# Isomorpfishm/SINGA

Measured on AMD Instinct MI355X. Metric: protein-ligand graphs/sec GAN step (G+D fwd+bwd); scatter-TP kernel HBM GB/s, higher is better.
Workload: dtype f32

## Files before the change

### __graft_entry__.py

```python
import os
import subprocess
import sys

ROOT = os.path.dirname(os.path.abspath(__file__))
if ROOT not in sys.path:
    sys.path.insert(0, ROOT)

SRC = os.path.join(ROOT, "singa_amd", "csrc", "singa_hip.hip")
LIB = os.path.join(ROOT, "singa_amd", "lib", "libsinga_hip.so")


def build() -> None:
    os.makedirs(os.path.dirname(LIB), exist_ok=True)
    deps = [SRC, os.path.join(ROOT, "singa_amd", "csrc", "so3_index.h"), os.path.join(ROOT, "include", "singa_hip.h"),
            os.path.join(ROOT, "include", "singa_hip_lab.h"), os.path.join(ROOT, "include", "singa_hip_gen.h"),
            os.path.join(ROOT, "include", "singa_hip_force.h"), os.path.join(ROOT, "include", "singa_hip_swor.h"),
            os.path.join(ROOT, "include", "singa_hip_stream.h"), os.path.join(ROOT, "include", "singa_hip_valence.h"),
            os.path.join(ROOT, "include", "singa_hip_beam.h"), os.path.join(ROOT, "include", "singa_hip_units.h"),
            os.path.join(ROOT, "include", "singa_hip_prefix.h"), os.path.join(ROOT, "include", "singa_hip_data.h"),
            os.path.join(ROOT, "include", "singa_hip_attn_tiles.h"), os.path.join(ROOT, "include", "singa_hip_bf16.h"),
            os.path.join(ROOT, "include", "singa_hip_dec_tiles.h")]
    if not os.path.exists(LIB) or any(os.path.getmtime(d) > os.path.getmtime(LIB) for d in deps):
        hipcc = os.environ.get("HIPCC", "/opt/rocm/bin/hipcc")
        cmd = [hipcc, "--offload-arch=gfx950", "-O3", "-std=c++17", "-shared", "-fPIC", "-o", LIB, SRC]
        subprocess.check_call(cmd)
    import torch
    import singa_amd
    from singa_amd import _capi
    _capi.bind(LIB)


def smoke() -> None:
    import numpy as np
    import torch

    build()
    from oracle import singa_oracle as O
    from singa_amd import graph as G
    from singa_amd.config import load_config
    from singa_amd.model.GAN import SINGA
    from tests.helpers import golden, state_from_spec

    assert torch.cuda.is_available(), "smoke() needs a GPU"
    L = 2
    dev = "cuda:0"
    sd = state_from_spec(f"singa_L{L}")
    z = golden(f"singa_L{L}_B3.npz")
    names = ["3wi2_4tpp", "4agq_5a7b", "5cp5_4nue"]
    batch = G.collate([G.load_npz(os.path.join(ROOT, "tests", "golden", f"graph_{n}.npz"), with_lap=False) for n in names])
    batch.nodes[G.PA]["lap_pe"], batch.nodes[G.LA]["lap_pe"] = torch.tensor(z["lap_p"]), torch.tensor(z["lap_l"])
    batch.extras["edge_rot_mat"] = {k: torch.tensor(z[f"rot_{k}"]) for k in ("pp", "ll", "lp")}
    batch.extras["knn"] = {G.PA: torch.tensor(z["knn_p"]), G.LA: torch.tensor(z["knn_l"])}
    batch = batch.to(dev)
    model = SINGA(load_config(lmax=L), device=dev)
    model.load_state_dict(sd, strict=False)
    model.eval()
    logits = model(batch)
    loss = torch.nn.functional.cross_entropy(logits, batch["ligand_data"]["smiIndices_tgt"].reshape(-1))
    loss.backward()
    torch.cuda.synchronize()
    og = O.collate([O.load_graph_npz(os.path.join(ROOT, "tests", "golden", f"graph_{n}.npz")) for n in names])
    rots = {k: torch.as_tensor(z[f"rot_{k}"]) for k in ("pp", "ll", "lp")}
    with torch.no_grad():
        ref = O.singa_forward(sd, og, rots, L, torch.as_tensor(z["knn_p"]), torch.as_tensor(z["knn_l"]),
                              torch.as_tensor(z["lap_p"]), torch.as_tensor(z["lap_l"]))
    err = float((logits.detach().cpu().double() - ref.double()).norm() / ref.double().norm())
    gn = float(torch.sqrt(sum((p.grad.double() ** 2).sum() for p in model.parameters() if p.grad is not None)))
    print(f"smoke: loss {float(loss):.6f} (reference {float(z['loss']):.6f}), logits rel err vs oracle {err:.2e}, "
          f"grad norm {gn:.4f} (reference {float(z['grad_total']):.4f})")
    assert err < 1e-4, err
    assert abs(gn - float(z["grad_total"])) < 1e-4 * float(z["grad_total"])


if __name__ == "__main__":
    build()
    if len(sys.argv) > 1 and sys.argv[1] == "smoke":
        smoke()
```

### singa_amd/_capi.py

```python
import ctypes as C

P = C.c_void_p
I32 = C.c_int
I64 = C.c_int64
F32 = C.c_float


class Seg(C.Structure):
    _fields_ = [("ptr", P), ("ld", I64), ("rows", C.c_int32)]


SegArr = Seg * 3


class Gemm(C.Structure):
    _fields_ = [("a", P), ("b", P), ("c", P), ("bias", P), ("lda", I64), ("ldb", I64), ("ldc", I64), ("I", C.c_int32),
                ("J", C.c_int32), ("R", C.c_int32), ("a_group", C.c_int32), ("b_group", C.c_int32), ("c_group", C.c_int32),
                ("a_group_ld", I64), ("b_group_ld", I64), ("c_group_ld", I64), ("c_split_stride", I64), ("mask", P),
                ("addend", P), ("relu", C.c_int32), ("asum", P), ("asum_stride", I64)]


class CGemm(C.Structure):
    _fields_ = [("a", P), ("b", P), ("c", P), ("lda", I64), ("ldb", I64), ("ldc", I64), ("a_im", I64), ("b_im", I64),
                ("c_im", I64), ("c_split_stride", I64), ("I", C.c_int32), ("J", C.c_int32), ("R", C.c_int32),
# ... 107 lines not shown
    "singa_smiles_rule_host": ([P, P, P, I32, P, P], I32),
}
GEN_EXPORTS = tuple(_GEN_SIGS)

_FORCE_SIGS = {
    "singa_sample_token_forced": ([P, P, P, P, P, I32, I32, I32, I32, F32, I32, F32, I32, I32] + [P] * 12, I32),
}
FORCE_EXPORTS = tuple(_FORCE_SIGS)

U64 = C.c_uint64
_SWOR_SIGS = {
    "singa_swor_noise_host": ([U64, P, P, P, I32, P, P, P], I32),
    "singa_swor_work": ([I32, I32], C.c_longlong),
    "singa_swor_expand": ([P, P, P, P, I32, I32, I32, I32, I32, F32, U64, P, I32] + [P] * 8 + [P], I32),
    "singa_swor_select": ([P, P, P, P, P, I32, I32, I32, I32, I32, I32, I32] + [P] * 13 + [P], I32),
    "singa_swor_follow": ([P] * 8 + [I32] * 6 + [I64] * 4 + [P], I32),
}
SWOR_EXPORTS = tuple(_SWOR_SIGS)

_STREAM_SIGS = {
    "singa_dec_self_attn_rows": ([P] * 10 + [I32, I32, P, F32, P], I32),
    "singa_sample_token_stream": ([P] * 6 + [I32, I32, I32, I32, I32, F32, I32, F32, I32, I32] + [P] * 7 + [P], I32),
    "singa_stream_refill": ([I32] * 8 + [P] * 8 + [P], I32),
    "singa_stream_refill_host": ([I32] * 8 + [P] * 8, I32),
}
STREAM_EXPORTS = tuple(_STREAM_SIGS)

_VALENCE_SIGS = {
    "singa_sample_token_valence": ([P] * 7 + [I32, I32, I32, I32, I32, F32, I32, F32, I32, I32] + [P] * 12 + [P], I32),
    "singa_valence_rule_host": ([P] * 5 + [I32] + [P] * 3, I32),
}
VALENCE_EXPORTS = tuple(_VALENCE_SIGS)

_BEAM_SIGS = {
    "singa_beam_work": ([I32, I32], C.c_longlong),
    "singa_beam_expand": ([P] * 5 + [I32] * 5 + [P] * 5 + [P], I32),
    "singa_beam_select": ([P] * 4 + [I32] * 7 + [P] * 18 + [P], I32),
}
BEAM_EXPORTS = tuple(_BEAM_SIGS)

_UNITS_SIGS = {
    "singa_edge_mlp_units_fwd": ([P] * 13 + [I32, I32, I32, I32, P], I32),
    "singa_edge_mlp_units_bwd": ([P] * 8 + [I32, I32, I32, P], I32),
}
UNITS_EXPORTS = tuple(_UNITS_SIGS)

_PREFIX_SIGS = {
    "singa_sample_token_stream_forced": ([P] * 7 + [I32, I32, I32, I32, I32, F32, I32, F32, I32, I32] + [P] * 10 + [P], I32),
    "singa_swor_expand_forced": ([P, P, P, P, I32, I32, I32, I32, I32, F32, U64, P, I32] + [P] * 9 + [P], I32),
    "singa_forced_beam_expand": ([P] * 5 + [I32] * 5 + [P] * 6 + [P], I32),
}
PREFIX_EXPORTS = tuple(_PREFIX_SIGS)


class CollateField(C.Structure):
    _fields_ = [("src", P), ("dst", P), ("axis", C.c_int32), ("width", C.c_int32), ("kind", C.c_int32), ("base_axis", C.c_int32)]


_DATA_SIGS = {
    "singa_collate_batch": ([P, I32, I32, P, P, P, C.POINTER(CollateField), I32, C.POINTER(I64), P], I32),
}
DATA_EXPORTS = tuple(_DATA_SIGS)

_ATTN_TILES_SIGS = {
    "singa_attn_tiles": ([P, I64, I64, P, P, I32, I32, I32, P], I32),
    "singa_attn_tiled_fwd": (_SIGS["singa_attn_fwd"][0][:-1] + [P, P], I32),
    "singa_attn_tiled_bwd": (_SIGS["singa_attn_bwd"][0][:-1] + [P, P, P], I32),
}
ATTN_TILES_EXPORTS = tuple(_ATTN_TILES_SIGS)

_BF16_SIGS = {
    "singa_gemm_bf16": (_SIGS["singa_gemm_f32"][0], I32),
    "singa_cgemm_bf16": (_SIGS["singa_cgemm3m_f32"][0], I32),
}
BF16_EXPORTS = tuple(_BF16_SIGS)

_DEC_TILES_SIGS = {
    "singa_dec_tile_self_attn": ([P] * 10 + [I32, I32, I32, I32, P, F32, P], I32),
    "singa_dec_tile_cross_attn": (_SIGS["singa_dec_cross_attn"][0], I32),
    "singa_dec_tile_ffn": (_SIGS["singa_dec_ffn"][0], I32),
}
DEC_TILES_EXPORTS = tuple(_DEC_TILES_SIGS)


def bind(path):
    import torch
    lib = C.CDLL(path)
    for name, (args, res) in list(_SIGS.items()) + list(_LAB_SIGS.items()) + list(_GEN_SIGS.items()) + \
            list(_FORCE_SIGS.items()) + list(_SWOR_SIGS.items()) + list(_STREAM_SIGS.items()) + list(_VALENCE_SIGS.items()) + \
            list(_BEAM_SIGS.items()) + list(_UNITS_SIGS.items()) + list(_PREFIX_SIGS.items()) + list(_DATA_SIGS.items()) + \
            list(_ATTN_TILES_SIGS.items()) + list(_BF16_SIGS.items()) + list(_DEC_TILES_SIGS.items()):
        fn = getattr(lib, name)
        fn.argtypes = args
        fn.restype = res
    return lib


def segs(items):
    arr = SegArr()
    for i, (p, ld, rows) in enumerate(items):
        arr[i].ptr, arr[i].ld, arr[i].rows = p, ld, rows
    return arr, len(items)


def check(lib, code, what):
    if code != 0:
        raise RuntimeError(f"{what} failed ({code}): {lib.singa_last_error_string().decode()}")
```

### singa_amd/csrc/singa_hip.hip

```cpp
#include <hip/hip_runtime.h>
#include <hip/hip_ext.h>

#include <math.h>
#include <stdint.h>
#include <stdio.h>
#include <string.h>
#include <type_traits>

#include "../../include/singa_hip.h"
#include "../../include/singa_hip_lab.h"
#include "../../include/singa_hip_gen.h"
#include "../../include/singa_hip_force.h"
#include "../../include/singa_hip_swor.h"
#include "../../include/singa_hip_stream.h"
#include "../../include/singa_hip_valence.h"
#include "../../include/singa_hip_beam.h"
#include "../../include/singa_hip_units.h"
#include "../../include/singa_hip_attn_tiles.h"
#include "../../include/singa_hip_prefix.h"
#include "../../include/singa_hip_data.h"
#include "../../include/singa_hip_bf16.h"
#include "../../include/singa_hip_dec_tiles.h"
#include "so3_index.h"

namespace {

thread_local char g_err[256] = "ok";

int fail(int code, const char* msg) {
    snprintf(g_err, sizeof(g_err), "%s", msg);
    return code;
}

int check_launch(const char* what) {
    hipError_t e = hipGetLastError();
    if (e != hipSuccess) {
        snprintf(g_err, sizeof(g_err), "%s: %s", what, hipGetErrorString(e));
        return (int)e;
    }
    return SINGA_OK;
}

struct ProfRec {
    hipEvent_t a, b;
    int E, N, tag;
};
constexpr int PROF_CAP = 8192;
ProfRec g_prof[PROF_CAP];
int g_prof_n = 0;
bool g_prof_on = false;
unsigned long long* g_stamp_buf = nullptr;
int g_stamp_cap = 0;
__global__ void stamp_kernel(unsigned long long* dst) { *dst = (unsigned long long)wall_clock64(); }
int g_prof_edges_hint = 0;

#ifndef SINGA_KEEP_VGPR
#define SINGA_KEEP_VGPR(x) __asm__ volatile("" : "+v"(x))
#endif

#define SINGA_LAUNCH(tag_, E_, N_, kern, grid, block, st, ...)                                                   \
    do {                                                                                                          \
        if (g_prof_on && g_prof_n < PROF_CAP) {                                                                   \
            ProfRec& r_ = g_prof[g_prof_n++];                                                                     \
            (void)hipEventCreate(&r_.a);                                                                          \
            (void)hipEventCreate(&r_.b);                                                                          \
            r_.E = (E_);                                                                                          \
            r_.N = (N_);                                                                                          \
            r_.tag = (tag_);                                                                                      \
            hipExtLaunchKernelGGL(kern, grid, block, 0, (st), r_.a, r_.b, 0, __VA_ARGS__);                        \
        } else if (g_stamp_buf && 2 * (g_prof_n + 2) <= g_stamp_cap && g_prof_n + 1 < PROF_CAP) {                 \
            if (g_prof_n == 0) {                                                                                  \
                g_prof[0].a = g_prof[0].b = nullptr;                                                              \
                g_prof[0].E = g_prof[0].N = g_prof[0].tag = 0;                                                    \
                hipLaunchKernelGGL(stamp_kernel, dim3(1), dim3(1), 0, (st), g_stamp_buf);                         \
                hipLaunchKernelGGL(stamp_kernel, dim3(1), dim3(1), 0, (st), g_stamp_buf + 1);                     \
                g_prof_n = 1;                                                                                     \
            }                                                                                                     \
            ProfRec& r_ = g_prof[g_prof_n];                                                                       \
            r_.a = r_.b = nullptr;                                                                                \
            r_.E = (E_);                                                                                          \
            r_.N = (N_);                                                                                          \
            r_.tag = (tag_);                                                                                      \
            hipLaunchKernelGGL(stamp_kernel, dim3(1), dim3(1), 0, (st), g_stamp_buf + 2 * g_prof_n);              \
            hipLaunchKernelGGL(kern, grid, block, 0, (st), __VA_ARGS__);                                          \
            hipLaunchKernelGGL(stamp_kernel, dim3(1), dim3(1), 0, (st), g_stamp_buf + 2 * g_prof_n + 1);          \
            ++g_prof_n;                                                                                           \
        } else                                                                                                    \
            hipLaunchKernelGGL(kern, grid, block, 0, (st), __VA_ARGS__);                                          \
    } while (0)

__device__ __forceinline__ int xcd_range_id(int vb, int n8) { return (vb & 7) * (n8 >> 3) + (vb >> 3); }
constexpr int MAX_J = 2300;
__device__ float g_J[MAX_J];
int g_lmax_init = -1;

__host__ __device__ constexpr int j_off(int l) {
    int s = 0;
    for (int i = 0; i < l; ++i) s += (2 * i + 1) * (2 * i + 1);
    return s;
}

struct Segs {
    const float* p[3];
    long long ld[3];
    int rows[3];
// ... 8380 lines not shown
    const int64_t* nbase = bases + (long long)f.base_axis * (B + 1);
    int slot = -1;
    long long soff = 0, nb = 0;
    for (long long w = w0 + threadIdx.x; w < wend; w += COLLATE_THREADS) {
        const unsigned wu = (unsigned)w;
        const unsigned r = width == 1 ? wu : wu / width;
        const unsigned col = wu - r * width;
        int sl = slot;
        if (sl < 0) {
            int lo = 0, hi = B;
            while (hi - lo > 1) {
                const int mid = (lo + hi) >> 1;
                if (sb[mid] <= (long long)r) lo = mid; else hi = mid;
            }
            sl = lo;
        } else {
            while ((long long)r >= sb[sl + 1]) ++sl;
        }
        if (sl != slot) {
            slot = sl;
            soff = aoff[collate_clamp_id(ids[sl], G)] - sb[sl];
            nb = f.kind == SINGA_COLLATE_WIDEN_BASE ? (long long)nbase[sl] : 0;
        }
        const long long si = (soff + (long long)r) * width + col;
        if (f.kind == SINGA_COLLATE_COPY32)
            ((uint32_t*)f.dst)[w] = ((const uint32_t*)f.src)[si];
        else if (f.kind == SINGA_COLLATE_SLOT)
            ((long long*)f.dst)[w] = (long long)sl;
        else
            ((long long*)f.dst)[w] = (long long)((const int32_t*)f.src)[si] + nb;
    }
}
#endif
}

int singa_collate_batch(const int32_t* ids, int B, int G, const int64_t* offsets, int64_t* bases, int32_t* status,
                        const singa_collate_field_t* fields, int n_fields, const int64_t* totals, void* stream) {
    const char* name = "collate_batch";
    if (!ids || !offsets || !bases || !status || !totals || (!fields && n_fields > 0)) return fail_at(SINGA_E_NULL, name, "null pointer");
    if (B < 1 || B > SINGA_COLLATE_MAX_B) return fail_at(SINGA_E_SHAPE, name, "B must be in [1, 2048]");
    if (G < 1) return fail_at(SINGA_E_SHAPE, name, "G >= 1 graphs in the store");
    if (n_fields < 0 || n_fields > SINGA_COLLATE_MAX_FIELDS) return fail_at(SINGA_E_SHAPE, name, "at most 32 fields");
    if (((uintptr_t)ids & 3) || ((uintptr_t)offsets & 7) || ((uintptr_t)bases & 7) || ((uintptr_t)status & 3))
        return fail_at(SINGA_E_SHAPE, name, "misaligned ids / offsets / bases / status");
    if (totals[SINGA_COLLATE_AXES - 1] != B) return fail_at(SINGA_E_SHAPE, name, "totals[6] must be B (width mismatch)");
    for (int a = 0; a < SINGA_COLLATE_AXES; ++a)
        if (totals[a] < 0) return fail_at(SINGA_E_SHAPE, name, "negative total");
    CollateArgs A;
    memset(&A, 0, sizeof(A));
    long long blocks = 0;
    for (int i = 0; i < n_fields; ++i) {
        const singa_collate_field_t& f = fields[i];
        if (f.axis < 0 || f.axis >= SINGA_COLLATE_AXES) return fail_at(SINGA_E_SHAPE, name, "field axis outside [0, 7)");
        if (f.width < 1) return fail_at(SINGA_E_SHAPE, name, "field width must be >= 1 (width mismatch)");
        if (f.kind < 0 || f.kind > SINGA_COLLATE_SLOT) return fail_at(SINGA_E_SHAPE, name, "field kind outside [0, 4)");
        if (f.kind == SINGA_COLLATE_WIDEN_BASE && (f.base_axis < 0 || f.base_axis > 1))
            return fail_at(SINGA_E_SHAPE, name, "base_axis must be 0 or 1");
        const long long items = (long long)totals[f.axis] * f.width;
        if (items == 0) continue;
        if (items >= (1LL << 31)) return fail_at(SINGA_E_SHAPE, name, "a field of 2^31 or more items");
        if (!f.dst || (!f.src && f.kind != SINGA_COLLATE_SLOT)) return fail_at(SINGA_E_NULL, name, "null field pointer");
        if (((uintptr_t)f.src & 3) || ((uintptr_t)f.dst & (f.kind == SINGA_COLLATE_COPY32 ? 3 : 7)))
            return fail_at(SINGA_E_SHAPE, name, "misaligned field pointer");
        A.f[A.n] = f;
        if (f.kind != SINGA_COLLATE_WIDEN_BASE) A.f[A.n].base_axis = 0;
        A.items[A.n] = items;
        A.blk0[A.n] = (int)blocks;
        blocks += (items + COLLATE_CHUNK - 1) / COLLATE_CHUNK;
        ++A.n;
    }
    A.blk0[A.n] = (int)blocks;
#ifdef SINGA_EMUL
    return fail_at(SINGA_E_SHAPE, name, "not part of the emulation build");
#else
    hipStream_t st = (hipStream_t)stream;
    hipLaunchKernelGGL(collate_plan_kernel, dim3(1), dim3(COLLATE_SCAN), 0, st, ids, B, G, offsets, bases, status);
    if (blocks > 0)
        hipLaunchKernelGGL(collate_copy_kernel, dim3((unsigned)blocks), dim3(COLLATE_THREADS), 0, st, A, ids, B, G, offsets,
                           (const int64_t*)bases);
    return check_launch(name);
#endif
}

}
```

### singa_amd/model/CProMG.py

```python
import math
import os

import numpy as np
import torch
import torch.nn as nn
import torch.nn.functional as F
from torch.nn import BatchNorm1d, Conv1d, Dropout, Embedding, LayerNorm, Sequential

from .. import ops
from ..nn import Linear


class ShiftedSoftplus(nn.Module):
    def __init__(self, device="cuda"):
        super().__init__()
        self.shift = math.log(2.0)

    def forward(self, x):
        return F.softplus(x) - self.shift


class GaussianSmearing(nn.Module):
    def __init__(self, start=0.0, stop=10.0, num_gaussians=50, device="cuda"):
        super().__init__()
        offset = torch.linspace(start, stop, num_gaussians, device=device)
        self.coeff = -0.5 / (offset[1] - offset[0]).item() ** 2
        self.register_buffer("offset", offset)

    def forward(self, dist):
        dist = dist.view(-1, 1) - self.offset.view(1, -1)
        return torch.exp(self.coeff * torch.pow(dist, 2))


class DenseMap:

    def __init__(self, batch, batch_size, mx=None):
        inside = batch < batch_size
        bc = batch.clamp(max=batch_size)
        num = torch.zeros(batch_size + 1, dtype=torch.int64, device=batch.device).index_add_(0, bc, torch.ones_like(batch))
        num = num[:batch_size]
        self.B = batch_size
        self.mx = int(num.max()) if mx is None else int(mx)
        start = num.cumsum(0) - num
        self.ptr = torch.cat([start, start[-1:] + num[-1:]])
        trash = batch_size * self.mx
        bi = batch.clamp(max=batch_size - 1)
        self.idx = torch.where(inside, torch.arange(batch.numel(), device=batch.device) - start[bi] + bi * self.mx,
                               torch.full_like(batch, trash))
        self.gidx = torch.where(inside, self.idx, torch.zeros_like(self.idx))
        mask = torch.zeros(trash + 1, dtype=torch.bool, device=batch.device)
        mask[self.idx] = True
        self.mask = mask[:trash].view(batch_size, self.mx)
        self.pad_mask = ~self.mask.unsqueeze(1)

    def tensors(self):
        return [self.idx, self.gidx, self.mask, self.pad_mask]

    def dense(self, x):
        out = x.new_zeros((self.B * self.mx + 1,) + tuple(x.shape[1:]))
        out = out.index_copy(0, self.idx, x)
        return out[:self.B * self.mx].view(self.B, self.mx, *x.shape[1:])

    def gather(self, dense_flat):
        return dense_flat.index_select(0, self.gidx)


def to_dense_batch(x, batch, batch_size):
    dm = DenseMap(batch, batch_size)
    return dm.dense(x), dm.mask, dm.idx


def knn_graph(pos, k, batch, batch_size, dm=None):
    dm = dm or DenseMap(batch, batch_size)
    return ops.knn_graph(pos, k, batch, dm.ptr, dm.mx)


class KnnEdges:

    def __init__(self, pos, knn_ei, smear, cap=None, n_real=None):
        N = pos.shape[0]
        dev = pos.device
        valid = (knn_ei[0] >= 0) & (knn_ei[1] >= 0)
        a, b = knn_ei[0].clamp(min=0), knn_ei[1].clamp(min=0)
        ln = (pos[a] - pos[b]).norm(dim=1)
        sentinel = N * N
        fwd = torch.where(valid, a * N + b, torch.full_like(a, sentinel))
        bwd = torch.where(valid, b * N + a, torch.full_like(a, sentinel))
        skey, perm = torch.sort(torch.cat([fwd, bwd]))
        new = torch.ones_like(skey, dtype=torch.bool)
        new[1:] = skey[1:] != skey[:-1]
        gid = torch.cumsum(new, 0) - 1
        triple = ((~new[2:] & ~new[1:-1] & (skey[2:] != sentinel)).any() if skey.numel() > 2
                  else torch.zeros((), dtype=torch.bool, device=dev))
        n_groups, last, triple = torch.stack([gid[-1] + 1, skey[-1], triple.to(gid.dtype)]).tolist()
        n_edges = n_groups - (1 if last == sentinel else 0)
        ukey = torch.zeros(n_groups, dtype=torch.int64, device=dev).scatter_(0, gid, skey)[:n_edges]
        ln2 = torch.cat([ln, ln])[perm]
        if not triple:
            nxt = torch.cat([ln2[1:], ln2[-1:]])
            prv = torch.cat([ln2[:1], ln2[:-1]])
            has_next = torch.cat([~new[1:], new.new_zeros(1)])
            mean = torch.where(new, torch.where(has_next, 0.5 * (ln2 + nxt), ln2), 0.5 * (prv + ln2))
            ln = torch.zeros(n_groups, device=dev).scatter_(0, gid, mean)[:n_edges]
        else:
            cnt = torch.zeros(n_groups, device=dev).index_add_(0, gid, torch.ones_like(ln2))[:n_edges]
            ln = torch.zeros(n_groups, device=dev).index_add_(0, gid, ln2)[:n_edges] / cnt
        row, col = ukey // N, ukey % N
        fused = ln.is_cuda and smear.offset.numel() == 64
        ea = None if fused else smear(ln)
        self.n_edges = n_edges + N
        if cap is not None:
            extra = cap - self.n_edges
            nd = N - n_real
            if extra < 0 or nd < 2:
                raise OverflowError(f"KnnEdges: {self.n_edges} edges do not fit the capacity {cap}")
            i = torch.arange(extra, device=dev)
            ps = (i * nd) // max(extra, 1)
            row = torch.cat([row, n_real + ps])
            col = torch.cat([col, n_real + (ps + 1 + i % (nd - 1)) % nd])
            if not fused:
                ea = torch.cat([ea, ea.new_zeros(extra, ea.shape[1])])
        loop = torch.arange(N, device=dev)
        bounds = torch.arange(N + 1, device=dev)
        if ln.is_cuda:
            E0 = row.shape[0]
            seg_ptr = torch.searchsorted(row, bounds)
            order = torch.empty(E0 + N, dtype=torch.int64, device=dev)
            order[torch.arange(E0, device=dev) + row] = torch.arange(E0, device=dev)
            order[seg_ptr[1:] + loop] = E0 + loop
            row, col = torch.cat([row, loop]), torch.cat([col, loop])
            self.row, self.col = row[order], col[order]
            seg32 = seg_ptr.to(torch.int32)
            if fused:
                self.attr = ops.knn_edge_attr(ln, seg32, E0, n_edges, smear.offset, smear.coeff)
            else:
                deg = ops.segment_sum_rows(ea.contiguous(), seg32)
                self.attr = torch.cat([-ea, deg], 0)[order].contiguous()
        else:
            deg = torch.zeros(N, ea.shape[1], device=dev).index_add_(0, row, ea)
            row, col = torch.cat([row, loop]), torch.cat([col, loop])
            attr = torch.cat([-ea, deg], 0)
            order = torch.argsort(row, stable=True)
            self.row, self.col, self.attr = row[order], col[order], attr[order].contiguous()
        self.row_ptr = torch.searchsorted(self.row, bounds).to(torch.int32)
        self.row32, self.col32 = self.row.to(torch.int32), self.col.to(torch.int32)
        eperm = torch.argsort(self.col32 if ln.is_cuda else self.col, stable=True)
        self.eperm = eperm.to(torch.int32)
        self.col_ptr = torch.searchsorted(self.col[eperm], bounds).to(torch.int32)
        self.N = N
        self.unit_a, self.unit_b = self._units(ukey, n_real, bool(triple))

    def _units(self, ukey, n_real, repeats):
        row, col = self.row, self.col
        E, N = row.shape[0], self.N
        idx = torch.arange(E, device=row.device)
        if repeats or ukey.numel() == 0:
            single = torch.ones_like(row, dtype=torch.bool)
        else:
            single = row == col
            if n_real is not None:
                single |= torch.maximum(row, col) >= n_real
        mate = torch.where(single, idx, torch.searchsorted(ukey, col * N + row) + col)
        first = single | (row < col)
        slot = torch.where(first, torch.cumsum(first, 0) - 1, E)
        both = torch.stack([idx, mate], 1).to(torch.int32)
        units = torch.full((E + 1, 2), -1, dtype=torch.int32, device=row.device).index_copy_(0, slot, both)
        return units[:E, 0].contiguous(), units[:E, 1].contiguous()

    def tensors(self):
        return [self.row, self.col, self.attr, self.row_ptr, self.row32, self.col32, self.eperm, self.col_ptr, self.unit_a,
                self.unit_b]


def set_precision(module, precision):
    ops.check_precision(precision)
    for m in module.modules():
        if hasattr(type(m), "precision"):
            m.precision = precision


class MultiHeadAttention(nn.Module):
    precision = "f32"

    def __init__(self, hidden_channels, edge_channels, key_channels, num_heads=1, device="cuda"):
        super().__init__()
        assert hidden_channels % num_heads == 0 and key_channels % num_heads == 0
        self.num_heads = num_heads
        self.k_lin = Conv1d(hidden_channels, key_channels, 1, groups=num_heads, bias=False, device=device)
        self.q_lin = Conv1d(hidden_channels, key_channels, 1, groups=num_heads, bias=False, device=device)
        self.v_lin = Conv1d(hidden_channels, hidden_channels, 1, groups=num_heads, bias=False, device=device)
        kh, vh = key_channels // num_heads, hidden_channels // num_heads
        self.weight_k_net = Sequential(Linear(edge_channels, kh, device=device), ShiftedSoftplus(), Linear(kh, kh, device=device))
        self.weight_k_lin = Linear(kh, kh, device=device)
        self.weight_v_net = Sequential(Linear(edge_channels, vh, device=device), ShiftedSoftplus(), Linear(vh, vh, device=device))
        self.weight_v_lin = Linear(vh, vh, device=device)
        self.centroid_lin = Linear(hidden_channels, hidden_channels, device=device)
        self.act = ShiftedSoftplus()
        self.out_transform = Linear(hidden_channels, hidden_channels, device=device)
        self.layer_norm = LayerNorm(hidden_channels, device=device)

    def _edge_mlp(self, net, x):
        return net[2](ops.bias_ssp(ops.linear(x, net[0].weight, precision=self.precision), net[0].bias))

    def forward(self, node_attr, edges: KnnEdges):
        N = node_attr.size(0)
        h_keys, h_queries, h_values = ops.grouped_linear3(node_attr, self.k_lin.weight, self.q_lin.weight, self.v_lin.weight,
                                                          self.num_heads, self.precision)
        scale = 1.0 / math.sqrt(h_keys.size(-1))
        if edges.attr.shape[1] == 64 and self.weight_k_net[0].out_features == 32 and self.weight_v_net[0].out_features == 64:
            W_k, W_v = ops.edge_mlp_pair(edges.attr, (self.weight_k_net[0], self.weight_k_net[2]),
                                         (self.weight_v_net[0], self.weight_v_net[2]),
                                         units=(edges.unit_a, edges.unit_b))
        else:
            W_k = self._edge_mlp(self.weight_k_net, edges.attr)
            W_v = self._edge_mlp(self.weight_v_net, edges.attr)
        qp = ops.linear_nn(h_queries, self.weight_k_lin.weight, self.precision)
        cterm = ops.rowdot_bias(h_queries, self.weight_k_lin.bias, scale)
        qk_ij = ops.edge_logits(qp, W_k, h_keys, cterm, edges, scale)
        alpha = ops.segment_softmax(qk_ij, edges.row_ptr, 0.0)
        S = ops.gather_wsum(alpha, W_v, h_values, edges)
        aggr_msg = ops.linear(S, self.weight_v_lin.weight, self.weight_v_lin.bias, self.precision).view(N, -1)
        out = ops.bias_ssp(ops.linear_add(node_attr, self.centroid_lin.weight, None, aggr_msg, self.precision),
                           self.centroid_lin.bias)
        return ops.layer_norm_residual(self.out_transform(out), None, self.layer_norm)


def _uses_k19(module, key_channels, hidden_channels):
    return key_channels // module.num_heads == 32 and hidden_channels // module.num_heads == 64


def _dense_attention(module, Q, K, V, attn_mask, key_channels, hidden_channels, tiles=None):
    B, heads = Q.size(0), module.num_heads
    dk, dv = key_channels // heads, hidden_channels // heads
    scale = 1.0 / math.sqrt(dk)
# ... 324 lines not shown
```

### singa_amd/ops.py

```python
import ctypes
import math
import warnings

import torch

warnings.filterwarnings("ignore", message=".*preferred_blas_library is an experimental feature.*")

from . import _capi, _lib, so3


PROFILE_ON = False


def profile_start(in_graph=False):
    global PROFILE_ON, _STAMPS
    PROFILE_ON = True
    if in_graph:
        _STAMPS = torch.zeros(2 * 8192 + 2, dtype=torch.int64, device="cuda")
        _chk(_lib.lib().singa_prof_stamps(_p(_STAMPS), _STAMPS.numel()), "singa_prof_stamps")
    else:
        _chk(_lib.lib().singa_prof_enable(1), "singa_prof_enable")


_STAMPS = None
# ... 261 lines not shown
            ctx.save_for_backward(y, row_ptr)
            return y
        _chk(_lib.lib().singa_segment_softmax_fwd(_p(x), _p(row_ptr), _p(y), N, x.shape[1], eps, ctx.dense, _stream()),
             "singa_segment_softmax_fwd")
        ctx.save_for_backward(y, row_ptr)
        return y

    @staticmethod
    def backward(ctx, gy):
        y, row_ptr = ctx.saved_tensors
        gy = gy.contiguous()
        gx = torch.empty_like(y)
        N = row_ptr.numel() - 1
        if y.shape[0] == 0:
            return gx, None, None
        _chk(_lib.lib().singa_segment_softmax_bwd(_p(y), _p(gy), _p(row_ptr), _p(gx), N, y.shape[1], ctx.dense, _stream()),
             "singa_segment_softmax_bwd")
        return gx, None, None


def segment_softmax(x, row_ptr, eps):
    return _SegmentSoftmax.apply(x, row_ptr, eps)


class _SegmentWSum(torch.autograd.Function):
    @staticmethod
    def forward(ctx, w, v, row_ptr):
        w, v = w.contiguous(), v.contiguous()
        _dev(w, v, row_ptr)
        E, H, F = v.shape
        N = row_ptr.numel() - 1
        ctx.save_for_backward(w, v, row_ptr)
        if E == 0:
            return torch.zeros(N, H, F, device=v.device, dtype=torch.float32)
        out = torch.empty(N, H, F, device=v.device, dtype=torch.float32)
        _chk(_lib.lib().singa_segment_wsum_fwd(_p(w), _p(v), _p(row_ptr), _p(out), N, H, F, _stream()),
             "singa_segment_wsum_fwd")
        return out

    @staticmethod
    def backward(ctx, g):
        w, v, row_ptr = ctx.saved_tensors
        g = g.contiguous()
        E, H, F = v.shape
        N = row_ptr.numel() - 1
        gw, gv = torch.empty_like(w), torch.empty_like(v)
        if E == 0:
            return gw, gv, None
        _chk(_lib.lib().singa_segment_wsum_bwd(_p(g), _p(w), _p(v), _p(row_ptr), _p(gw), _p(gv), N, H, F, _stream()),
             "singa_segment_wsum_bwd")
        return gw, gv, None


def segment_sum_rows(v, row_ptr):
    v = v.detach()
    _dev(v, row_ptr)
    E, F = v.shape
    N = row_ptr.numel() - 1
    out = torch.empty(N, 1, F, device=v.device, dtype=torch.float32)
    w = torch.ones(max(E, 1), 1, device=v.device, dtype=torch.float32)
    _chk(_lib.lib().singa_segment_wsum_fwd(_p(w), _p(v), _p(row_ptr), _p(out), N, 1, F, _stream()), "singa_segment_wsum_fwd")
    return out.view(N, F)


def knn_edge_attr(ln, seg_ptr, E0, n_real, offset, coeff):
    ln, offset = ln.detach().contiguous(), offset.detach().contiguous()
    _dev(ln, seg_ptr, offset)
    N = seg_ptr.numel() - 1
    out = torch.empty(E0 + N, offset.numel(), device=ln.device, dtype=torch.float32)
    _chk(_lib.lib().singa_knn_edge_attr(_p(ln), _p(seg_ptr), int(n_real), _p(offset), float(coeff), _p(out), N, offset.numel(),
                                        _stream()), "singa_knn_edge_attr")
    return out


def knn_graph(pos, k, batch, ptr, max_nodes):
    pos = pos.detach().to(torch.float32).contiguous()
    b32 = batch.to(torch.int32).contiguous()
    _dev(pos, b32)
    p64 = ptr.to(device=pos.device, dtype=torch.int64).contiguous()
    N = pos.shape[0]
    out = torch.empty(2, N * k, dtype=torch.int64, device=pos.device)
    _chk(_lib.lib().singa_knn_graph(_p(pos), _p(b32), _p(p64), p64.numel() - 1, N, int(k), int(max_nodes), _p(out[0]), _p(out[1]),
                                    _stream()), "singa_knn_graph")
    return out


def segment_wsum(w, v, row_ptr):
    return _SegmentWSum.apply(w, v, row_ptr)


_grid_cache = {}


def _grid_factors(L, M, m_primary, device):
    key = (L, M, m_primary, str(device))
    if key not in _grid_cache:
        _grid_cache[key] = tuple(torch.tensor(t, dtype=torch.float32, device=device).contiguous()
                                 for t in so3.s2_grid_factors(L, M, m_primary))
    return _grid_cache[key]


def _s2_edge_src(h0, h1, h2, gate_off, x_off, C, L, M):
    seg, n = _segs3((h0[:, x_off:], h1, h2), so3.layout(L, M).seg_rows, C)
    return (seg, n, _p(h0[:, gate_off:]), h0.stride(0)) + tuple(_p(t) for t in _grid_factors(L, M, True, h0.device))


def _s2_node_src(x, gate, L):
    seg, n = _capi.segs([(x.data_ptr(), x.shape[1] * x.shape[2], x.shape[1])])
    return (seg, n, _p(gate), gate.stride(0)) + tuple(_p(t) for t in _grid_factors(L, L, False, x.device))


def _s2_fwd_edge(h0, h1, h2, gate_off, x_off, C, L, M):
    E = h0.shape[0]
    out = torch.empty(E, so3.layout(L, M).KR * C, device=h0.device, dtype=torch.float32)
    if E > 0:
        _chk(_lib.lib().singa_s2act_sep_fwd(*_s2_edge_src(h0, h1, h2, gate_off, x_off, C, L, M), _p(out), E, C, L, _stream()),
             "singa_s2act_sep_fwd")
    return out


def _s2_fwd_node(x, gate, L):
    out = torch.empty_like(x)
    if x.shape[0] > 0:
        _chk(_lib.lib().singa_s2act_sep_fwd(*_s2_node_src(x, gate, L), _p(out), x.shape[0], x.shape[2], L, _stream()),
             "singa_s2act_sep_fwd(node)")
    return out


def _s2_bwd(src, g, E, KC, C, L, what):
    gx = torch.empty(E, KC, device=g.device, dtype=torch.float32)
    gg = torch.empty(E, C, device=g.device, dtype=torch.float32)
    if E > 0:
        _chk(_lib.lib().singa_s2act_sep_bwd(*src, _p(g), _p(gx), _p(gg), E, C, L, _stream()), what)
    return gx, gg


def _s2_bwd_seg(src, g, gseg, g_gate, E, C, L):
    if E > 0:
        _chk(_lib.lib().singa_s2act_sep_bwd_seg(*src, _p(g), gseg, _p(g_gate), g_gate.stride(0), E, C, L, _stream()),
             "singa_s2act_sep_bwd_seg")


class _S2ActEdge(torch.autograd.Function):

    @staticmethod
    def forward(ctx, h0, h1, h2, gate_off, x_off, C, L, M):
        h0, h1, h2 = _rows(h0), _rows(h1), _rows(h2)
        _dev(h0, h1, h2)
        ctx.save_for_backward(h0, h1, h2)
        ctx.cfg = (gate_off, x_off, C, L, M)
        return _s2_fwd_edge(h0, h1, h2, gate_off, x_off, C, L, M)

    @staticmethod
    def backward(ctx, g):
        h0, h1, h2 = ctx.saved_tensors
        gate_off, x_off, C, L, M = ctx.cfg
        lay = so3.layout(L, M)
        gx, gg = _s2_bwd(_s2_edge_src(h0, h1, h2, *ctx.cfg), g.contiguous(), h0.shape[0], lay.KR * C, C, L,
                         "singa_s2act_sep_bwd")
        n0, n1 = lay.seg_rows[0] * C, lay.seg_rows[1] * C
        g0 = torch.zeros_like(h0)
        g0[:, gate_off:gate_off + C] = gg
        g0[:, x_off:] = gx[:, :n0]
        return g0, gx[:, n0:n0 + n1], gx[:, n0 + n1:], None, None, None, None, None


# ... 1839 lines not shown
```

Baseline: 899.9.

## Build KNN edge CSR structures with native HIP kernels instead of torch ops

Replaces the torch-based construction of symmetric KNN edge lists (sort, searchsorted, unique and mate pairing) with a chain of custom HIP kernels. These count slots, scan offsets, place entries, rank columns within rows, pad edges and resolve mates. The aim is to cut the many small torch launches and sorts done per graph batch. The cost is one host sync to read back the edge count. The code falls back to the torch path when inputs are malformed or do not match the expected shapes.

```diff
diff --git a/__graft_entry__.py b/__graft_entry__.py
--- a/__graft_entry__.py
+++ b/__graft_entry__.py
@@ -19,7 +19,7 @@
             os.path.join(ROOT, "include", "singa_hip_beam.h"), os.path.join(ROOT, "include", "singa_hip_units.h"),
             os.path.join(ROOT, "include", "singa_hip_prefix.h"), os.path.join(ROOT, "include", "singa_hip_data.h"),
             os.path.join(ROOT, "include", "singa_hip_attn_tiles.h"), os.path.join(ROOT, "include", "singa_hip_bf16.h"),
-            os.path.join(ROOT, "include", "singa_hip_dec_tiles.h")]
+            os.path.join(ROOT, "include", "singa_hip_dec_tiles.h"), os.path.join(ROOT, "include", "singa_hip_knn_edges.h")]
     if not os.path.exists(LIB) or any(os.path.getmtime(d) > os.path.getmtime(LIB) for d in deps):
         hipcc = os.environ.get("HIPCC", "/opt/rocm/bin/hipcc")
         cmd = [hipcc, "--offload-arch=gfx950", "-O3", "-std=c++17", "-shared", "-fPIC", "-o", LIB, SRC]
diff --git a/include/singa_hip_knn_edges.h b/include/singa_hip_knn_edges.h
--- /dev/null
+++ b/include/singa_hip_knn_edges.h
@@ -0,0 +1,19 @@
+#ifndef SINGA_HIP_KNN_EDGES_H
+#define SINGA_HIP_KNN_EDGES_H
+#include <stdint.h>
+#ifdef __cplusplus
+extern "C" {
+#endif
+long long singa_knn_edges_work(int N, int n_real);
+
+int singa_knn_edges_count(const long long* knn_row, const long long* knn_col, int N, int k, int n_real, int32_t* nb, int32_t* mate,
+                          int32_t* work, int32_t* seg, int32_t* ubase, long long* head, void* stream);
+
+int singa_knn_edges_fill(const int32_t* nb, const int32_t* mate, const float* ln, int32_t* work, int32_t* seg, int32_t* ubase, int N,
+                         int k, int n_real, long long n0, long long extra, int32_t* esrc, int32_t* ecol, long long* row, long long* col,
+                         int32_t* row_ptr, int32_t* row32, int32_t* col32, int32_t* eperm, int32_t* col_ptr, int32_t* unit_a,
+                         int32_t* unit_b, float* lnm, void* stream);
+#ifdef __cplusplus
+}
+#endif
+#endif
diff --git a/singa_amd/_capi.py b/singa_amd/_capi.py
--- a/singa_amd/_capi.py
+++ b/singa_amd/_capi.py
@@ -213,6 +213,13 @@
 }
 DEC_TILES_EXPORTS = tuple(_DEC_TILES_SIGS)
 
+_KNN_EDGES_SIGS = {
+    "singa_knn_edges_work": ([I32, I32], C.c_longlong),
+    "singa_knn_edges_count": ([P, P, I32, I32, I32] + [P] * 6 + [P], I32),
+    "singa_knn_edges_fill": ([P] * 6 + [I32, I32, I32, C.c_longlong, C.c_longlong] + [P] * 12 + [P], I32),
+}
+KNN_EDGES_EXPORTS = tuple(_KNN_EDGES_SIGS)
+
 
 def bind(path):
     import torch
@@ -220,7 +227,8 @@
     for name, (args, res) in list(_SIGS.items()) + list(_LAB_SIGS.items()) + list(_GEN_SIGS.items()) + \
             list(_FORCE_SIGS.items()) + list(_SWOR_SIGS.items()) + list(_STREAM_SIGS.items()) + list(_VALENCE_SIGS.items()) + \
             list(_BEAM_SIGS.items()) + list(_UNITS_SIGS.items()) + list(_PREFIX_SIGS.items()) + list(_DATA_SIGS.items()) + \
-            list(_ATTN_TILES_SIGS.items()) + list(_BF16_SIGS.items()) + list(_DEC_TILES_SIGS.items()):
+            list(_ATTN_TILES_SIGS.items()) + list(_BF16_SIGS.items()) + list(_DEC_TILES_SIGS.items()) + \
+            list(_KNN_EDGES_SIGS.items()):
         fn = getattr(lib, name)
         fn.argtypes = args
         fn.restype = res
diff --git a/singa_amd/csrc/singa_hip.hip b/singa_amd/csrc/singa_hip.hip
--- a/singa_amd/csrc/singa_hip.hip
+++ b/singa_amd/csrc/singa_hip.hip
@@ -21,6 +21,7 @@
 #include "../../include/singa_hip_data.h"
 #include "../../include/singa_hip_bf16.h"
 #include "../../include/singa_hip_dec_tiles.h"
+#include "../../include/singa_hip_knn_edges.h"
 #include "so3_index.h"
 
 namespace {
@@ -8567,4 +8568,338 @@
 #endif
 }
 
-}
+namespace {
+#ifndef SINGA_EMUL
+constexpr int KE_UNSTRUCTURED = 1, KE_DUPLICATE = 2, KE_RANGE = 4;
+constexpr int KE_LCAP = 256;
+
+__global__ __launch_bounds__(256) void ke_slots_kernel(const long long* __restrict__ krow, const long long* __restrict__ kcol,
+                                                        int total, int k, int n_real, int* __restrict__ nb, int* status) {
+    for (int s = blockIdx.x * 256 + threadIdx.x; s < total; s += gridDim.x * 256) {
+        const long long r = krow[s], c = kcol[s];
+        const int i = s / k;
+        int out = -1, bad = 0;
+        if (r != -1 && r != i) bad |= KE_UNSTRUCTURED;
+        if (r >= 0 && c >= 0) {
+            if (c >= n_real || c == i || i >= n_real) bad |= KE_RANGE;
+            else out = (int)c;
+        }
+        nb[s] = bad ? -1 : out;
+        if (bad) atomicOr(status, bad);
+    }
+}
+
+__global__ __launch_bounds__(256) void ke_count_kernel(const int* __restrict__ nb, int N, int k, int* __restrict__ mate, int* deg,
+                                                        int* hi, int* __restrict__ outcnt, int* status) {
+    const int lane = threadIdx.x & 63;
+    const int i = blockIdx.x * 4 + (threadIdx.x >> 6);
+    if (i >= N) return;
+    const int base = i * k;
+    const int myj = lane < k ? nb[base + lane] : -1;
+    int mymate = -2;
+    bool dup = false;
+    for (int s = 0; s < k; ++s) {
+        const int js = __shfl(myj, s, 64);
+        if (js < 0) continue;
+        const int v = lane < k ? nb[js * k + lane] : -1;
+        const unsigned long long m = __ballot(v == i);
+        if (__popcll(__ballot(myj == js)) > 1) dup = true;
+        if (lane == s) mymate = m ? js * k + (__ffsll((long long)m) - 1) : -1;
+    }
+    if (lane < k) mate[base + lane] = mymate;
+    const bool valid = myj >= 0;
+    if (mymate == -1) {
+        atomicAdd(&deg[myj], 1);
+        if (i > myj) atomicAdd(&hi[myj], 1);
+    }
+    const int oc = __popcll(__ballot(valid)), oh = __popcll(__ballot(valid && myj > i));
+    if (lane == 0) {
+        outcnt[i] = oc;
+        if (oc) atomicAdd(&deg[i], oc);
+        if (oh) atomicAdd(&hi[i], oh);
+        if (dup) atomicOr(status, KE_DUPLICATE);
+    }
+}
+
+__global__ __launch_bounds__(1024) void ke_scan_kernel(const int* __restrict__ a, const int* __restrict__ b, int n, int* __restrict__ sa,
+                                                        int* __restrict__ sb, const int* status, long long* head) {
+    __shared__ long long la[1024], lb[1024];
+    const int t = threadIdx.x;
+    const int per = (n + 1023) / 1024;
+    const long long b0 = (long long)t * per;
+    const int beg = (int)(b0 < n ? b0 : n), end = beg + per < n ? beg + per : n;
+    long long va = 0, vb = 0;
+    for (int x = beg; x < end; ++x) {
+        if (a) va += a[x];
+        if (b) vb += b[x] + 1;
+    }
+    la[t] = va, lb[t] = vb;
+    __syncthreads();
+    for (int off = 1; off < 1024; off <<= 1) {
+        const long long pa = t >= off ? la[t - off] : 0, pb = t >= off ? lb[t - off] : 0;
+        __syncthreads();
+        la[t] += pa, lb[t] += pb;
+        __syncthreads();
+    }
+    long long ra = la[t] - va, rb = lb[t] - vb;
+    for (int x = beg; x < end; ++x) {
+        if (a) sa[x] = (int)ra, ra += a[x];
+        if (b) sb[x] = (int)rb, rb += b[x] + 1;
+    }
+    if (t == 1023) {
+        if (a) sa[n] = (int)la[1023];
+        if (b) sb[n] = (int)lb[1023];
+        if (head) head[0] = la[1023], head[1] = *status;
+    }
+}
+
+__global__ __launch_bounds__(256) void ke_entries_kernel(const int* __restrict__ nb, const int* __restrict__ mate,
+                                                          const int* __restrict__ seg, const int* __restrict__ outcnt, int* cur, int N,
+                                                          int k, int* __restrict__ esrc, int* __restrict__ ecol) {
+    const int lane = threadIdx.x & 63;
+    const int i = blockIdx.x * 4 + (threadIdx.x >> 6);
+    if (i >= N) return;
+    const int s = i * k + lane;
+    const int myj = lane < k ? nb[s] : -1;
+    const bool valid = myj >= 0;
+    const unsigned long long vm = __ballot(valid);
+    if (valid) {
+        const int at = seg[i] + __popcll(vm & ((1ull << lane) - 1ull));
+        esrc[at] = s, ecol[at] = myj;
+        if (mate[s] == -1) {
+            const int p = seg[myj] + outcnt[myj] + atomicAdd(&cur[myj], 1);
+            esrc[p] = ~s, ecol[p] = i;
+        }
+    }
+}
+
+__device__ __forceinline__ int ke_rank(const int* cols, int m, int c) {
+    int r = 0;
+    for (int x = 0; x < m; ++x) r += cols[x] < c;
+    return r;
+}
+
+__global__ __launch_bounds__(256) void ke_rows_kernel(const int* __restrict__ esrc, const int* __restrict__ ecol,
+                                                       const int* __restrict__ mate, const float* __restrict__ ln,
+                                                       const int* __restrict__ seg, const int* __restrict__ ubase, int rows,
+                                                       long long* __restrict__ row, long long* __restrict__ col, int* __restrict__ row_ptr,
+                                                       int* __restrict__ col_ptr, int* __restrict__ row32, int* __restrict__ col32,
+                                                       int* __restrict__ eperm, int* __restrict__ unit_a, int* __restrict__ unit_b,
+                                                       float* __restrict__ lnm) {
+    __shared__ int lds[4][KE_LCAP];
+    const int w = threadIdx.x >> 6, lane = threadIdx.x & 63;
+    const int i = blockIdx.x * 4 + w;
+    const bool live = i < rows;
+    const int b = live ? seg[i] : 0, m = live ? seg[i + 1] - b : 0;
+    const bool in_lds = m <= KE_LCAP;
+    if (in_lds)
+        for (int x = lane; x < m; x += 64) lds[w][x] = ecol[b + x];
+    __syncthreads();
+    int nl = 0;
+    for (int x0 = 0; x0 < m; x0 += 64) {
+        const int e = x0 + lane;
+        const bool on = e < m;
+        const int c = on ? ecol[b + e] : 0x7fffffff;
+        const int r = in_lds ? ke_rank(lds[w], m, c) : ke_rank(ecol + b, m, c);
+        nl += __popcll(__ballot(on && c < i));
+        if (on) {
+            const int code = esrc[b + e];
+            const int s = code >= 0 ? code : ~code;
+            float len = ln[s];
+            if (code >= 0) {
+                const int mt = mate[s];
+                if (mt >= 0) len = 0.5f * (len + ln[mt]);
+            }
+            const int p = b + i + r;
+            row[p] = i, col[p] = c, row32[p] = i, col32[p] = c;
+            lnm[b + r] = len;
+        }
+    }
+    if (live && lane == 0) {
+        const int p = b + m + i;
+        row[p] = i, col[p] = i, row32[p] = i, col32[p] = i;
+        row_ptr[i] = b + i, col_ptr[i] = b + i;
+        eperm[b + i + nl] = p;
+        const int u = ubase[i] + (m - nl);
+        unit_a[u] = p, unit_b[u] = p;
+    }
+}
+
+__device__ __forceinline__ long long ke_pad_start(long long p, long long extra, int nd) { return (p * extra + nd - 1) / nd; }
+
+__global__ __launch_bounds__(256) void ke_tail_ptr_kernel(int N, int n_real, long long n0, long long extra, int* __restrict__ seg,
+                                                           int* ubase, int* __restrict__ row_ptr, int* __restrict__ col_ptr) {
+    const int nd = N - n_real;
+    const int u_real = ubase[n_real];
+    for (int p = blockIdx.x * 256 + threadIdx.x; p <= nd; p += gridDim.x * 256) {
+        const long long st = nd > 0 ? ke_pad_start(p, extra, nd) : 0;
+        if (p > 0) seg[n_real + p] = (int)(n0 + st), ubase[n_real + p] = (int)(u_real + st + p);
+        row_ptr[n_real + p] = (int)(n0 + st + n_real + p);
+        if (p == nd) col_ptr[N] = (int)(n0 + st + N);
+    }
+}
+
+__global__ __launch_bounds__(256) void ke_pad_edges_kernel(int N, int n_real, long long n0, long long extra, const int* __restrict__ ubase,
+                                                            long long* __restrict__ row, long long* __restrict__ col,
+                                                            int* __restrict__ row32, int* __restrict__ col32, int* __restrict__ unit_a,
+                                                            int* __restrict__ unit_b, int* pcnt) {
+    const int nd = N - n_real;
+    const int u_real = ubase[n_real];
+    const long long total = extra + nd;
+    for (long long t = blockIdx.x * 256LL + threadIdx.x; t < total; t += gridDim.x * 256LL) {
+        if (t < extra) {
+            const long long ps = (t * nd) / extra;
+            const int a = n_real + (int)ps, q = (int)((ps + 1 + t % (nd - 1)) % nd);
+            const long long p = n0 + t + a;
+            row[p] = a, col[p] = n_real + q, row32[p] = a, col32[p] = n_real + q;
+            const long long u = u_real + t + ps;
+            unit_a[u] = (int)p, unit_b[u] = (int)p;
+            atomicAdd(&pcnt[q], 1);
+        } else {
+            const int ps = (int)(t - extra), a = n_real + ps;
+            const long long nx = ke_pad_start(ps + 1, extra, nd);
+            const long long p = n0 + nx + a, u = u_real + nx + ps;
+            row[p] = a, col[p] = a, row32[p] = a, col32[p] = a;
+            unit_a[u] = (int)p, unit_b[u] = (int)p;
+        }
+    }
+}
+
+__global__ __launch_bounds__(256) void ke_pad_cols_kernel(int N, int n_real, long long n0, long long extra, const int* __restrict__ pbase,
+                                                           int E, int* __restrict__ eperm, int* __restrict__ col_ptr) {
+    const int nd = N - n_real, M = nd - 1;
+    const int lane = threadIdx.x & 63;
+    const int q = blockIdx.x * 4 + (threadIdx.x >> 6);
+    if (q >= nd) return;
+    const int start = (int)(n0 + n_real) + pbase[q];
+    if (lane == 0) col_ptr[n_real + q] = start;
+    int run = 0;
+    for (int p0 = 0; p0 < nd; p0 += 64) {
+        const int p = p0 + lane;
+        long long first = 0;
+        int cnt = 0;
+        if (p < nd && p != q) {
+            const long long A = ke_pad_start(p, extra, nd), B = ke_pad_start(p + 1, extra, nd);
+            const int r = (q - p + nd) % nd - 1;
+            first = A + ((r - (int)(A % M)) + M) % M;
+            cnt = first < B ? (int)((B - 1 - first) / M) + 1 : 0;
+        }
+        int inc = cnt;
+        for (int d = 1; d < 64; d <<= 1) {
+            const int v = __shfl_up(inc, d, 64);
+            if (lane >= d) inc += v;
+        }
+        const int at = start + run + (inc - cnt);
+        for (int t = 0; t < cnt && at + (p > q) + t < E; ++t) eperm[at + (p > q) + t] = (int)(n0 + first + (long long)t * M + n_real + p);
+        if (p == q && at < E) eperm[at] = (int)(n0 + ke_pad_start(q + 1, extra, nd) + n_real + q);
+        run += __shfl(inc, 63, 64);
+    }
+}
+
+__global__ __launch_bounds__(256) void ke_mates_kernel(const int* __restrict__ row32, const int* __restrict__ col32,
+                                                        const int* __restrict__ row_ptr, const int* __restrict__ ubase, int N, int n_pos,
+                                                        int E, int* __restrict__ eperm, int* __restrict__ unit_a, int* __restrict__ unit_b) {
+    const int utot = ubase[N];
+    for (int p = blockIdx.x * 256 + threadIdx.x; p < E; p += gridDim.x * 256) {
+        if (p >= utot) unit_a[p] = -1, unit_b[p] = -1;
+        if (p >= n_pos) continue;
+        const int r = row32[p], c = col32[p];
+        if (r == c) continue;
+        const int lo = row_ptr[c], end = row_ptr[c + 1] - 1;
+        int a = lo, z = end;
+        while (a < z) {
+            const int mid = (a + z) >> 1;
+            if (col32[mid] < r) a = mid + 1;
+            else z = mid;
+        }
+        if (a >= end) continue;
+        eperm[a + (r > c)] = p;
+        if (r < c) {
+            const int rb = row_ptr[r];
+            const int nlow = (row_ptr[r + 1] - rb - 1) - (ubase[r + 1] - ubase[r] - 1);
+            const int u = ubase[r] + (p - rb) - nlow;
+            if (u >= 0 && u < E) unit_a[u] = p, unit_b[u] = a;
+        }
+    }
+}
+#endif
+
+inline unsigned ke_grid(long long items, int per_block) {
+    const long long g = (items + per_block - 1) / per_block;
+    return (unsigned)(g < 1 ? 1 : g > 16384 ? 16384 : g);
+}
+}
+
+long long singa_knn_edges_work(int N, int n_real) {
+    if (N < 0 || n_real < 0 || n_real > N) return 0;
+    return 4LL * N + 2LL * (N - n_real) + 8;
+}
+
+int singa_knn_edges_count(const long long* knn_row, const long long* knn_col, int N, int k, int n_real, int32_t* nb, int32_t* mate,
+                          int32_t* work, int32_t* seg, int32_t* ubase, long long* head, void* stream) {
+    const char* name = "knn_edges_count";
+    if (!knn_row || !knn_col || !nb || !mate || !work || !seg || !ubase || !head) return fail_at(SINGA_E_NULL, name, "null pointer");
+    if (N <= 0 || k <= 0 || k > 64) return fail_at(SINGA_E_SHAPE, name, "N > 0 atoms and 1 <= k <= 64 slots per atom");
+    if (n_real < 0 || n_real > N) return fail_at(SINGA_E_SHAPE, name, "0 <= n_real <= N");
+    if ((long long)N * k >= (1LL << 31)) return fail_at(SINGA_E_SHAPE, name, "2^31 or more slots (positions are 32-bit)");
+#ifdef SINGA_EMUL
+    return fail_at(SINGA_E_SHAPE, name, "not part of the emulation build");
+#else
+    hipStream_t st = (hipStream_t)stream;
+    int *deg = work, *hi = work + N, *outcnt = work + 2LL * N, *status = work + 4LL * N + 2LL * (N - n_real) + 4;
+    hipLaunchKernelGGL(ke_slots_kernel, dim3(ke_grid((long long)N * k, 256)), dim3(256), 0, st, knn_row, knn_col, N * k, k, n_real, nb,
+                       status);
+    hipLaunchKernelGGL(ke_count_kernel, dim3((unsigned)((N + 3) / 4)), dim3(256), 0, st, (const int*)nb, N, k, mate, deg, hi, outcnt,
+                       status);
+    hipLaunchKernelGGL(ke_scan_kernel, dim3(1), dim3(1024), 0, st, (const int*)deg, (const int*)hi, N, seg, ubase, (const int*)status,
+                       head);
+    return check_launch(name);
+#endif
+}
+
+int singa_knn_edges_fill(const int32_t* nb, const int32_t* mate, const float* ln, int32_t* work, int32_t* seg, int32_t* ubase, int N,
+                         int k, int n_real, long long n0, long long extra, int32_t* esrc, int32_t* ecol, long long* row, long long* col,
+                         int32_t* row_ptr, int32_t* row32, int32_t* col32, int32_t* eperm, int32_t* col_ptr, int32_t* unit_a,
+                         int32_t* unit_b, float* lnm, void* stream) {
+    const char* name = "knn_edges_fill";
+    if (!nb || !mate || !work || !seg || !ubase || !row || !col || !row_ptr || !row32 || !col32 || !eperm || !col_ptr || !unit_a ||
+        !unit_b)
+        return fail_at(SINGA_E_NULL, name, "null pointer");
+    if (N <= 0 || k <= 0 || k > 64) return fail_at(SINGA_E_SHAPE, name, "N > 0 atoms and 1 <= k <= 64 slots per atom");
+    if (n_real < 0 || n_real > N) return fail_at(SINGA_E_SHAPE, name, "0 <= n_real <= N");
+    if ((long long)N * k >= (1LL << 31)) return fail_at(SINGA_E_SHAPE, name, "2^31 or more slots (positions are 32-bit)");
+    if (n0 < 0 || extra < 0 || n0 > 2LL * N * k) return fail_at(SINGA_E_SHAPE, name, "edge counts out of range");
+    if (n0 + extra + N >= (1LL << 31)) return fail_at(SINGA_E_SHAPE, name, "2^31 or more edges (positions are 32-bit)");
+    if (extra > 0 && N - n_real < 2) return fail_at(SINGA_E_SHAPE, name, "padding edges need two padding atoms");
+    if (n0 > 0 && (!ln || !esrc || !ecol || !lnm)) return fail_at(SINGA_E_NULL, name, "null pointer");
+#ifdef SINGA_EMUL
+    return fail_at(SINGA_E_SHAPE, name, "not part of the emulation build");
+#else
+    hipStream_t st = (hipStream_t)stream;
+    const int nd = N - n_real;
+    const int E = (int)(n0 + extra + N);
+    int *outcnt = work + 2LL * N, *cur = work + 3LL * N, *pcnt = work + 4LL * N, *pbase = pcnt + nd;
+    if (n0 > 0)
+        hipLaunchKernelGGL(ke_entries_kernel, dim3((unsigned)((N + 3) / 4)), dim3(256), 0, st, nb, mate, (const int*)seg,
+                           (const int*)outcnt, cur, N, k, esrc, ecol);
+    if (n_real > 0)
+        hipLaunchKernelGGL(ke_rows_kernel, dim3((unsigned)((n_real + 3) / 4)), dim3(256), 0, st, (const int*)esrc, (const int*)ecol, mate,
+                           ln, (const int*)seg, (const int*)ubase, n_real, row, col, row_ptr, col_ptr, row32, col32, eperm, unit_a,
+                           unit_b, lnm);
+    hipLaunchKernelGGL(ke_tail_ptr_kernel, dim3(ke_grid(nd + 1, 256)), dim3(256), 0, st, N, n_real, n0, extra, seg, ubase, row_ptr,
+                       col_ptr);
+    if (nd > 0) {
+        hipLaunchKernelGGL(ke_pad_edges_kernel, dim3(ke_grid(extra + nd, 256)), dim3(256), 0, st, N, n_real, n0, extra,
+                           (const int*)ubase, row, col, row32, col32, unit_a, unit_b, pcnt);
+        hipLaunchKernelGGL(ke_scan_kernel, dim3(1), dim3(1024), 0, st, (const int*)nullptr, (const int*)pcnt, nd, (int*)nullptr, pbase,
+                           (const int*)nullptr, (long long*)nullptr);
+        hipLaunchKernelGGL(ke_pad_cols_kernel, dim3((unsigned)((nd + 3) / 4)), dim3(256), 0, st, N, n_real, n0, extra,
+                           (const int*)pbase, E, eperm, col_ptr);
+    }
+    hipLaunchKernelGGL(ke_mates_kernel, dim3(ke_grid(E, 256)), dim3(256), 0, st, (const int*)row32, (const int*)col32,
+                       (const int*)row_ptr, (const int*)ubase, N, (int)(n0 + n_real), E, eperm, unit_a, unit_b);
+    return check_launch(name);
+#endif
+}
+
+}
diff --git a/singa_amd/model/CProMG.py b/singa_amd/model/CProMG.py
--- a/singa_amd/model/CProMG.py
+++ b/singa_amd/model/CProMG.py
@@ -77,12 +77,15 @@
 
 class KnnEdges:
 
-    def __init__(self, pos, knn_ei, smear, cap=None, n_real=None):
+    def __init__(self, pos, knn_ei, smear, cap=None, n_real=None, force_torch=False):
         N = pos.shape[0]
         dev = pos.device
-        valid = (knn_ei[0] >= 0) & (knn_ei[1] >= 0)
         a, b = knn_ei[0].clamp(min=0), knn_ei[1].clamp(min=0)
         ln = (pos[a] - pos[b]).norm(dim=1)
+        self.native = not force_torch and self._build_native(knn_ei, ln, smear, N, cap, n_real)
+        if self.native:
+            return
+        valid = (knn_ei[0] >= 0) & (knn_ei[1] >= 0)
         sentinel = N * N
         fwd = torch.where(valid, a * N + b, torch.full_like(a, sentinel))
         bwd = torch.where(valid, b * N + a, torch.full_like(a, sentinel))
@@ -150,6 +153,23 @@
         self.N = N
         self.unit_a, self.unit_b = self._units(ukey, n_real, bool(triple))
 
+    def _build_native(self, knn_ei, ln, smear, N, cap, n_real):
+        M = knn_ei.shape[1] if knn_ei.dim() == 2 else 0
+        if not (ln.is_cuda and knn_ei.is_cuda and smear.offset.numel() == 64 and ln.dtype == torch.float32
+                and knn_ei.dtype == torch.int64 and knn_ei.dim() == 2 and knn_ei.shape[0] == 2 and N > 0 and M > 0 and M % N == 0
+                and M // N <= ops.KNN_EDGES_MAX_K and (cap is None) == (n_real is None) and M < 2 ** 31
+                and (2 * M + N if cap is None else cap) < 2 ** 31):
+            return False
+        out = ops.knn_edges(knn_ei, ln, N, M // N, n_real, cap)
+        if out is None:
+            return False
+        self.N, self.n_edges = N, out["n_edges"]
+        self.row, self.col, self.row_ptr, self.col_ptr = out["row"], out["col"], out["row_ptr"], out["col_ptr"]
+        self.row32, self.col32, self.eperm = out["row32"], out["col32"], out["eperm"]
+        self.unit_a, self.unit_b = out["unit_a"], out["unit_b"]
+        self.attr = ops.knn_edge_attr(out["ln"], out["seg_ptr"], out["E0"], out["n_real_edges"], smear.offset, smear.coeff)
+        return True
+
     def _units(self, ukey, n_real, repeats):
         row, col = self.row, self.col
         E, N = row.shape[0], self.N
diff --git a/singa_amd/ops.py b/singa_amd/ops.py
--- a/singa_amd/ops.py
+++ b/singa_amd/ops.py
@@ -367,6 +367,64 @@
     out = torch.empty(2, N * k, dtype=torch.int64, device=pos.device)
     _chk(_lib.lib().singa_knn_graph(_p(pos), _p(b32), _p(p64), p64.numel() - 1, N, int(k), int(max_nodes), _p(out[0]), _p(out[1]),
                                     _stream()), "singa_knn_graph")
+    return out
+
+
+KNN_EDGES_MAX_K = 64
+
+
+def knn_edges(knn_ei, ln, N, k, n_real=None, cap=None, alloc=None):
+    if knn_ei.dtype != torch.int64 or ln.dtype != torch.float32:
+        raise ValueError(f"knn_edges: knn_ei must be int64 and ln float32, got {knn_ei.dtype} and {ln.dtype}")
+    N, k = int(N), int(k)
+    if N <= 0 or not 1 <= k <= KNN_EDGES_MAX_K:
+        raise ValueError(f"knn_edges: N > 0 atoms and 1 <= k <= {KNN_EDGES_MAX_K} slots per atom, got N = {N}, k = {k}")
+    if knn_ei.dim() != 2 or tuple(knn_ei.shape) != (2, N * k) or tuple(ln.shape) != (N * k,):
+        raise ValueError(f"knn_edges: knn_ei must be [2, N * k] = [2, {N * k}] and ln [N * k], got {tuple(knn_ei.shape)} and "
+                         f"{tuple(ln.shape)}")
+    if (n_real is None) != (cap is None):
+        raise ValueError("knn_edges: n_real and cap go together")
+    nr = N if n_real is None else int(n_real)
+    if not 0 <= nr <= N:
+        raise ValueError(f"knn_edges: n_real = {nr} outside [0, {N}]")
+    if N * k >= 2 ** 31 or (2 * N * k + N if cap is None else int(cap)) >= 2 ** 31:
+        raise ValueError("knn_edges: 2^31 or more slots or edges (positions are 32-bit)")
+    _dev(ln)
+    if knn_ei.device != ln.device:
+        raise RuntimeError(f"knn_edges: knn_ei on {knn_ei.device}, ln on {ln.device}")
+    knn_ei, ln = knn_ei.contiguous(), ln.detach().contiguous()
+    dev, lib = ln.device, _lib.lib()
+    i32 = dict(dtype=torch.int32, device=dev)
+    work = torch.zeros(int(lib.singa_knn_edges_work(N, nr)), **i32)
+    nb, mate = torch.empty(N * k, **i32), torch.empty(N * k, **i32)
+    ubase, head = torch.empty(N + 1, **i32), torch.empty(2, dtype=torch.int64, device=dev)
+    new = alloc or (lambda name, shape, dtype: torch.empty(shape, dtype=dtype, device=dev))
+    seg = new("seg_ptr", (N + 1,), torch.int32)
+    _chk(lib.singa_knn_edges_count(_p(knn_ei[0]), _p(knn_ei[1]), N, k, nr, _p(nb), _p(mate), _p(work), _p(seg), _p(ubase), _p(head),
+                                   _stream()), "singa_knn_edges_count")
+    n0, status = head.tolist()
+    if status:
+        return None
+    n_edges = n0 + N
+    extra = 0
+    if cap is not None:
+        extra = int(cap) - n_edges
+        if extra < 0 or N - nr < 2:
+            raise OverflowError(f"KnnEdges: {n_edges} edges do not fit the capacity {cap}")
+    E = n_edges + extra
+    if E >= 2 ** 31:
+        raise ValueError("knn_edges: 2^31 or more edges (positions are 32-bit)")
+    esrc, ecol = torch.empty(n0, **i32), torch.empty(n0, **i32)
+    out = {"row": new("row", (E,), torch.int64), "col": new("col", (E,), torch.int64), "ln": new("ln", (n0,), torch.float32)}
+    for name in ("row_ptr", "col_ptr"):
+        out[name] = new(name, (N + 1,), torch.int32)
+    for name in ("row32", "col32", "eperm", "unit_a", "unit_b"):
+        out[name] = new(name, (E,), torch.int32)
+    _chk(lib.singa_knn_edges_fill(_p(nb), _p(mate), _p(ln), _p(work), _p(seg), _p(ubase), N, k, nr, n0, extra, _p(esrc), _p(ecol),
+                                  _p(out["row"]), _p(out["col"]), _p(out["row_ptr"]), _p(out["row32"]), _p(out["col32"]),
+                                  _p(out["eperm"]), _p(out["col_ptr"]), _p(out["unit_a"]), _p(out["unit_b"]), _p(out["ln"]), _stream()),
+         "singa_knn_edges_fill")
+    out.update(seg_ptr=seg, n_real_edges=n0, E0=n0 + extra, n_edges=n_edges)
     return out
 
 
```

New measurement: 905.3 (median of 6 runs). No clear change (+0.6%).
